# drprojects/superpoint_transformer

Hardware: AMD Instinct MI355X
Metric: Mpoints/s SPT fwd+bwd on S3DIS-scale NAG (higher is better)
Workload: dtype f32 (the reference's shipped matmul class - configs/train.yaml:60-61 `float32_matmul_precision: high` = TF32 / bf16x3 next to `precision: 32` - as bf16x3: matrix products on the bf16 pipe with split operands, attention and the backward of the fused layers and of the attention blocks' Linears hi*hi +

## Files before the change

include/spt_hip.h:

```cpp
#ifndef SPT_HIP_H
#define SPT_HIP_H

#include <stddef.h>
#include <stdint.h>

#ifdef __cplusplus
extern "C" {
#endif

typedef void* spt_stream_t;

enum spt_reduce_op {
  SPT_SUM = 0,
  SPT_MEAN = 1,
  SPT_MIN = 2,
  SPT_MAX = 3
};

typedef struct spt_gn_fwd_tables {
  const float* weight;
  const float* mean_scale;
  float eps;
  float* mean;
  float* rstd;
// ... 436 lines not shown
                                 float* gmean_scale, spt_stream_t stream);

int spt_fused_linear_supported(int K, int N);
int spt_fused_linear_use_split_bf16(int mode);
size_t spt_fused_linear_workspace_bytes(int K, int N);
int spt_fused_linear_fwd_f32(const float* x, int64_t r0, int64_t r1, int K, const float* W,
                             int N, const float* pre_am, const float* pre_scale,
                             const float* pre_bias, float pre_slope, float* h, double* total,
                             void* ws, size_t ws_bytes, spt_stream_t stream);
int spt_fused_linear_bwd_f32(const float* gy, const float* h, int64_t r0, int64_t r1, int N,
                             const float* am, const float* scale, const float* bias,
                             float slope, const float* c1, const float* c2, const float* c3,
                             const float* xprev, int K, const float* pre_am,
                             const float* pre_scale, const float* pre_bias, float pre_slope,
                             const float* W, float* gx, float* gW, int accumulate,
                             double* prev_total, void* ws, size_t ws_bytes, spt_stream_t stream);
int spt_fused_linear_pooled_supported(int K, int N);
int spt_fused_linear_pooled_supported_ex(int K, int N, int mode);
#define SPT_FMLP_BWD_REGISTER_STAGED 4
#define SPT_FMLP_H_BF16 8
#define SPT_FMLP_X_BF16 16
int spt_fused_linear_storage_supported(int K, int N);
int spt_fused_linear_bwd_use_dma(int on);
int spt_fused_linear_fwd_use_x3(int on);
int spt_fused_linear_fwd_ex_f32(const float* x, int64_t r0, int64_t r1, int K, const float* W,
                                int N, const float* pre_am, const float* pre_scale,
                                const float* pre_bias, float pre_slope, float* h, double* total,
                                int mode, void* ws, size_t ws_bytes, spt_stream_t stream);
int spt_fused_linear_bwd_ex_f32(const float* gy, const float* h, int64_t r0, int64_t r1, int N,
                                const float* am, const float* scale, const float* bias,
                                float slope, const float* c1, const float* c2, const float* c3,
                                const float* xprev, int K, const float* pre_am,
                                const float* pre_scale, const float* pre_bias, float pre_slope,
                                const float* W, float* gx, float* gW, int accumulate,
                                double* prev_total, int mode, void* ws, size_t ws_bytes,
                                spt_stream_t stream);
int spt_fused_linear_bwd_pooled_ex_f32(
    const float* gout, const int32_t* arg, const int32_t* perm, const int32_t* pos_seg,
    const float* h, int64_t p0, int64_t p1, int N, const float* am, const float* scale,
    const float* bias, float slope, const float* c1, const float* c2, const float* c3,
    const float* xprev, int K, const float* pre_am, const float* pre_scale, const float* pre_bias,
    float pre_slope, const float* W, float* gx, float* gW, int accumulate, double* prev_total,
    int mode, void* ws, size_t ws_bytes, spt_stream_t stream);
int spt_fused_linear_bwd_pooled_f32(
    const float* gout, const int32_t* arg, const int32_t* perm, const int32_t* pos_seg,
    const float* h, int64_t p0, int64_t p1, int N, const float* am, const float* scale,
// ... 116 lines not shown
```

superpoint_transformer_amd/_lib.py:

```python
import ctypes
import os

import torch

_HERE = os.path.dirname(os.path.abspath(__file__))
LIB_PATH = os.path.join(_HERE, "lib", "libspt_hip.so")

_c = ctypes
_i64 = _c.c_int64
_int = _c.c_int
_p = _c.c_void_p
_sz = _c.c_size_t
_f32 = _c.c_float
_f64 = _c.c_double

SIGNATURES = {
    "spt_version": (_int, []),
    "spt_last_error": (_c.c_char_p, []),
    "spt_csr_build_workspace_bytes": (_sz, [_i64, _i64]),
    "spt_csr_build": (_int, [_p, _i64, _i64, _p, _p, _p, _sz, _p]),
    "spt_csr_pos_seg": (_int, [_p, _i64, _i64, _p, _p]),
    "spt_csr_gather_i64_i32": (_int, [_p, _p, _i64, _p, _p]),
    "spt_segcsr_reduce_f32": (_int, [_int, _p, _p, _p, _i64, _i64, _int, _p, _p, _p]),
    "spt_segcsr_max_affine_f32": (_int, [_p, _p, _p, _i64, _i64, _int, _p, _p, _p, _f32, _p, _p, _p, _p]),
# ... 72 lines not shown
    "spt_spatial_order_workspace_bytes": (_sz, [_i64, _i64]),
    "spt_spatial_order": (_int, [_p, _i64, _f32, _p, _p, _p, _p, _sz, _p]),
    "spt_point_geof_csr_f32": (_int, [_p, _i64, _p, _p, _int, _int, _int, _p, _p]),
    "spt_vertical_edge_features_f32": (_int, [_p, _i64] + [_p] * 13 + [_p]),
    "spt_edge_affinity_features_f32": (_int, [_p, _i64, _int, _p, _p, _i64, _p, _p]),
    "spt_edge_affinity_features_bwd_f32": (_int, [_p, _p, _i64, _int, _p, _p, _i64, _p, _p]),
    "spt_scatter_pca_f32": (_int, [_p, _p, _p, _i64, _p, _p, _p]),
    "spt_neighbors_dense_to_csr_workspace_bytes": (_sz, [_i64]),
    "spt_neighbors_dense_to_csr": (_int, [_p, _i64, _int, _p, _p, _p, _p, _sz, _p]),
    "spt_horizontal_edge_features_f32": (_int, [_p, _i64, _i64, _p, _p, _p, _p, _p, _p, _p, _int,
                                                _p, _p, _p]),
    "spt_graphnorm_tables_f32": (_int, [_p, _int, _int, _p, _p, _f32, _p, _p, _p, _p, _p]),
    "spt_graphnorm_apply_f32": (_int, [_p, _p, _i64, _int, _int, _p, _p, _p, _f32, _p, _p]),
    "spt_graphnorm_bwd_stats_f32": (_int, [_p, _p, _p, _i64, _int, _int, _p, _p, _p, _f32, _p,
                                           _p, _sz, _p]),
    "spt_graphnorm_bwd_stats_sparse_workspace_bytes": (_sz, [_i64, _int, _int]),
    "spt_graphnorm_bwd_stats_sparse_f32": (_int, [_p, _p, _p, _p, _p, _i64, _i64, _int, _int, _p, _p,
                                                   _p, _f32, _p, _p, _sz, _p]),
    "spt_graphnorm_bwd_tables_f32": (_int, [_p, _int, _int, _p, _p, _p, _p, _p, _p, _p, _p, _p,
                                            _p, _p]),
    "spt_fused_linear_supported": (_int, [_int, _int]),
    "spt_fused_linear_use_split_bf16": (_int, [_int]),
    "spt_fused_linear_bwd_use_dma": (_int, [_int]),
    "spt_fused_linear_fwd_use_x3": (_int, [_int]),
    "spt_fused_linear_pooled_supported": (_int, [_int, _int]),
    "spt_fused_linear_bwd_pooled_f32": (_int, [_p, _p, _p, _p, _p, _i64, _i64, _int, _p, _p, _p, _f32,
                                               _p, _p, _p, _p, _int, _p, _p, _p, _f32, _p, _p, _p,
                                               _int, _p, _p, _sz, _p]),
    "spt_fused_linear_pooled_supported_ex": (_int, [_int, _int, _int]),
    "spt_fused_linear_fwd_ex_f32": (_int, [_p, _i64, _i64, _int, _p, _int, _p, _p, _p, _f32, _p, _p,
                                           _int, _p, _sz, _p]),
    "spt_fused_linear_bwd_ex_f32": (_int, [_p, _p, _i64, _i64, _int, _p, _p, _p, _f32, _p, _p, _p,
                                           _p, _int, _p, _p, _p, _f32, _p, _p, _p, _int, _p, _int, _p,
                                           _sz, _p]),
    "spt_fused_linear_bwd_pooled_ex_f32": (_int, [_p, _p, _p, _p, _p, _i64, _i64, _int, _p, _p, _p, _f32,
                                                  _p, _p, _p, _p, _int, _p, _p, _p, _f32, _p, _p, _p,
                                                  _int, _p, _int, _p, _sz, _p]),
    "spt_fused_linear_workspace_bytes": (_sz, [_int, _int]),
    "spt_fused_linear_fwd_runs_f32": (_int, [_p, _int, _p, _p, _p, _int, _int, _p, _int, _p, _p, _p,
                                             _f32, _p, _p, _int, _p, _sz, _p]),
    "spt_fused_linear_bwd_runs_f32": (_int, [_p, _p, _int, _p, _p, _p, _int, _int, _p, _p, _p, _f32,
                                             _p, _p, _p, _p, _int, _p, _p, _p, _f32, _p, _p, _p, _p,
                                             _int, _p, _sz, _p]),
    "spt_fused_linear_bwd_pooled_runs_f32": (_int, [_p, _p, _p, _p, _p, _int, _p, _p, _p, _int, _int,
                                                    _p, _p, _p, _f32, _p, _p, _p, _p, _int, _p, _p,
                                                    _p, _f32, _p, _p, _p, _p, _int, _p, _sz, _p]),
# ... 148 lines not shown
```

superpoint_transformer_amd/csrc/fused_mlp.hip:

```cpp
#include <math.h>
#include <stdlib.h>

#include "common.hpp"

namespace spt {
namespace fmlp {

typedef float f32x4 __attribute__((ext_vector_type(4)));
constexpr int WAVES = 4;
constexpr int TR = 16;
constexpr int MAX_BLOCKS = 1024;
constexpr int MAX_BWD_WAVES = 4096;

__device__ __forceinline__ double xg_sum_d(double v) {
  v += __shfl_xor(v, 16, 64);
  v += __shfl_xor(v, 32, 64);
  return v;
}
__device__ __forceinline__ void wave_sync_lds() {
  __builtin_amdgcn_fence(__ATOMIC_RELEASE, "wavefront");
  __builtin_amdgcn_wave_barrier();
  __builtin_amdgcn_fence(__ATOMIC_ACQUIRE, "wavefront");
}

// ... 1606 lines not shown
}

static int grid_for(int64_t rows, int per_cu) {
  const int64_t tiles = (rows + TR - 1) / TR;
  int64_t blocks = (tiles + WAVES - 1) / WAVES;
  const int64_t cap = 256 * per_cu;
  if (blocks > cap) blocks = cap;
  if (blocks < 1) blocks = 1;
  return (int)blocks;
}

}

bool fmlp_dma_supported(int K, int N);
int fmlp_dma_bwd_launch(bool pooled, bool lo, const float* gy, const float* h, FmlpRuns rt,
                        int64_t max_rows, int N, const float* am, const float* sc, const float* bs,
                        float slope, const float* c1, const float* c2, const float* c3,
                        const float* xprev, int K, const float* pam, const float* psc,
                        const float* pbs, float pslope, const float* W, float* gx,
                        float* gw_partial, double* pstat_partial, const int32_t* perm,
                        const int32_t* pos_seg, const float* gout, const int32_t* arg,
                        hipStream_t stream, bool s16 = false, int* gw_tabs = nullptr,
                        const float* x0 = nullptr, const float* fshift = nullptr,
                        float* fold_partial = nullptr, int K0 = 0);
bool fmlp_dma_fold_supported(int K0, int K, int N);
int fmlp_fold_len(int K, int K0);
}

using namespace spt;
using namespace spt::fmlp;

#define SPT_FMLP_SHAPES(X) X(3, 2) X(5, 2) X(8, 2) X(8, 4) X(16, 4) X(16, 8) X(17, 4) X(33, 4)

static std::atomic<int> g_fmlp_mode{1};
static inline int fmlp_mode_of(int mode) { return mode < 0 ? (int)g_fmlp_mode : (mode & 3); }
static std::atomic<int> g_fmlp_x3{[] { const char* e = getenv("SPT_FMLP_X3"); return e ? (atoi(e) != 0) : 1; }()};
extern "C" int spt_fused_linear_fwd_use_x3(int on) {
  const int prev = g_fmlp_x3;
  if (on >= 0) g_fmlp_x3 = on != 0;
  return prev;
}
static std::atomic<int> g_fmlp_dma{1};
static inline bool fmlp_dma_of(int mode) { return g_fmlp_dma != 0 && !(mode >= 0 && (mode & 4)); }
extern "C" int spt_fused_linear_bwd_use_dma(int on) {
  const int prev = g_fmlp_dma;
  if (on >= 0) g_fmlp_dma = on != 0;
  return prev;
}
// ... 304 lines not shown
    else if (g_fmlp_mode == 3)                                                                   \
      bwd_kernel_bf<a, b, false, NWB, false><<<grid, NWB * 64, 0, stream>>>(                     \
          gy, h, 0, 0, am, scale, bias, slope, c1, c2, c3, xprev, K, pre_am, pre_scale,          \
          pre_bias, pre_slope, W, nullptr, gwp, nullptr, rt);                                    \
    else if (g_fmlp_split_bf16 && gx)                                                            \
      bwd_kernel_bf<a, b, true, NWB, true><<<grid, NWB * 64, 0, stream>>>(                       \
          gy, h, 0, 0, am, scale, bias, slope, c1, c2, c3, xprev, K, pre_am, pre_scale,          \
          pre_bias, pre_slope, W, gx, gwp, pstp, rt);                                            \
    else if (g_fmlp_split_bf16)                                                                  \
      bwd_kernel_bf<a, b, false, NWB, true><<<grid, NWB * 64, 0, stream>>>(                      \
          gy, h, 0, 0, am, scale, bias, slope, c1, c2, c3, xprev, K, pre_am, pre_scale,          \
          pre_bias, pre_slope, W, nullptr, gwp, nullptr, rt);                                    \
    else if (gx)                                                                                 \
      bwd_kernel<a, b, true, NWV, big><<<grid, NWV * 64, 0, stream>>>(                           \
          gy, h, 0, 0, am, scale, bias, slope, c1, c2, c3, xprev, K, pre_am, pre_scale,          \
          pre_bias, pre_slope, W, gx, gwp, pstp, rt);                                            \
    else                                                                                         \
      bwd_kernel<a, b, false, NWV, big><<<grid, NWV * 64, 0, stream>>>(                          \
          gy, h, 0, 0, am, scale, bias, slope, c1, c2, c3, xprev, K, pre_am, pre_scale,          \
          pre_bias, pre_slope, W, nullptr, gwp, nullptr, rt);                                    \
  }
  float* fold_tabs = nullptr;
  float* fold_shift = nullptr;
  int per_run = 0;
  int gw_tabs = 0;
  const bool h16 = mode >= 0 && (mode & SPT_FMLP_H_BF16), x16 = mode >= 0 && (mode & SPT_FMLP_X_BF16);
  if (h16 || x16) {
    SPT_CHECK_ARG(g_fmlp_mode == 3 && h16 && spt_fused_linear_storage_supported(K, N) &&
                  (!x16 || K % 16 == 0),
                  "bf16 activation storage: bf16 matrix mode, a built shape, h stored as bf16");
#define XSP(a, b)                                                                                \
  if (pooled && k4 == a && nbk == b) {                                                           \
    constexpr bool big = (a * b >= 32);                                                          \
    constexpr int NWB = (a * b > 128) ? 4 : (big ? 8 : 4);                                       \
    gx_ = cap_grid(grid_for_nw(max_rows, (a * b > 128) ? 1 : (big ? ((a * b <= 32) ? 2 : 1) : 4), NWB), NWB); \
    nwv = NWB;                                                                                   \
    gw_tabs = gx_ * (fmlp_bf_wg_reduce(a, b, NWB) ? 1 : NWB);                                    \
    const dim3 grid((unsigned)gx_, (unsigned)nr);                                                \
    if (x16)                                                                                     \
      bwd_kernel_bf<a, b, true, NWB, false, true, false, true, true><<<grid, NWB * 64, 0, stream>>>( \
          nullptr, h, 0, 0, am, scale, bias, slope, c1, c2, c3, xprev, K, pre_am, pre_scale,     \
          pre_bias, pre_slope, W, gx, gwp, pstp, rt, perm, pos_seg, gout, arg);                  \
    else                                                                                         \
      bwd_kernel_bf<a, b, true, NWB, false, true, false, true, false><<<grid, NWB * 64, 0, stream>>>( \
          nullptr, h, 0, 0, am, scale, bias, slope, c1, c2, c3, xprev, K, pre_am, pre_scale,     \
          pre_bias, pre_slope, W, gx, gwp, pstp, rt, perm, pos_seg, gout, arg);                  \
// ... 4 lines not shown
    constexpr int NWV = big ? 8 : 4;                                                             \
    constexpr int NWB = (a * b > 128) ? 4 : NWV;                                                 \
    gx_ = cap_grid(grid_for_nw(max_rows, (a * b > 128) ? 1 : (big ? ((a * b <= 32) ? 2 : 1) : 4), NWB), NWB); \
    nwv = NWB;                                                                                   \
    gw_tabs = gx_ * (fmlp_bf_wg_reduce(a, b, NWB) ? 1 : NWB);                                    \
    const dim3 grid((unsigned)gx_, (unsigned)nr);                                                \
    if (gx && x16)                                                                               \
      bwd_kernel_bf<a, b, true, NWB, false, false, false, true, true><<<grid, NWB * 64, 0, stream>>>( \
          gy, h, 0, 0, am, scale, bias, slope, c1, c2, c3, xprev, K, pre_am, pre_scale,          \
          pre_bias, pre_slope, W, gx, gwp, pstp, rt);                                            \
    else if (gx)                                                                                 \
      bwd_kernel_bf<a, b, true, NWB, false, false, false, true, false><<<grid, NWB * 64, 0, stream>>>( \
          gy, h, 0, 0, am, scale, bias, slope, c1, c2, c3, xprev, K, pre_am, pre_scale,          \
          pre_bias, pre_slope, W, gx, gwp, pstp, rt);                                            \
    else if (x16)                                                                                \
      bwd_kernel_bf<a, b, false, NWB, false, false, false, true, true><<<grid, NWB * 64, 0, stream>>>( \
          gy, h, 0, 0, am, scale, bias, slope, c1, c2, c3, xprev, K, pre_am, pre_scale,          \
          pre_bias, pre_slope, W, nullptr, gwp, nullptr, rt);                                    \
    else                                                                                         \
      bwd_kernel_bf<a, b, false, NWB, false, false, false, true, false><<<grid, NWB * 64, 0, stream>>>( \
          gy, h, 0, 0, am, scale, bias, slope, c1, c2, c3, xprev, K, pre_am, pre_scale,          \
          pre_bias, pre_slope, W, nullptr, gwp, nullptr, rt);                                    \
  }
    if (x16 && gx && fmlp_dma_of(mode) && fmlp_dma_supported(K, N)) {
      per_run = fmlp_dma_bwd_launch(pooled, false, gy, h, rt, max_rows, N, am, scale, bias, slope, c1,
                                    c2, c3, xprev, K, pre_am, pre_scale, pre_bias, pre_slope, W, gx,
                                    gwp, pstp, perm, pos_seg, gout, arg, stream, true, &gw_tabs);
    } else {
      SPT_FMLP_ST_POOLED_SHAPES(XSP)
      SPT_FMLP_ST_SHAPES(XSD)
      per_run = gx_ * nwv;
    }
#undef XSP
#undef XSD
  } else if (fold_x0) {
    constexpr size_t FOLD_MAX_TABS = 1024;
    const int flen = fmlp_fold_len(K, fold_K0);
    SPT_CHECK_ARG((FOLD_MAX_TABS * ((size_t)N * K + flen) + FMLP_MAX_RUNS * FOLD_SHIFT_LD) * 4 <=
                  (size_t)MAX_BWD_WAVES * N * K * 4, "fold: tables do not fit the workspace");
    fold_tabs = gwp + FOLD_MAX_TABS * N * K;
    fold_shift = fold_tabs + FOLD_MAX_TABS * flen;
    fold_shift_kernel<<<num_graphs, 1024, 0, stream>>>(fold_x0, fold_K0, rt, fold_shift);
    if (fmlp_dma_of(mode) && fmlp_dma_fold_supported(fold_K0, K, N)) {
      per_run = fmlp_dma_bwd_launch(false, true, gy, h, rt, max_rows, N, am, scale, bias, slope, c1, c2,
                                    c3, xprev, K, pre_am, pre_scale, pre_bias, pre_slope, W, nullptr,
                                    gwp, pstp, nullptr, nullptr, nullptr, nullptr, stream, false,
                                    &gw_tabs, fold_x0, fold_shift, fold_tabs, fold_K0);
    } else if (fold_K0 == 18 && k4 == 8 && nbk == 2) {
      constexpr int NWB = 4;
      gx_ = cap_grid(grid_for_nw(max_rows, 4, NWB), NWB);
      nwv = NWB;
      gw_tabs = gx_;
      const dim3 grid((unsigned)gx_, (unsigned)nr);
      bwd_kernel_bf<8, 2, true, NWB, true, false, false, false, false, 18><<<grid, NWB * 64, 0, stream>>>(
          gy, h, 0, 0, am, scale, bias, slope, c1, c2, c3, xprev, K, pre_am, pre_scale, pre_bias,
          pre_slope, W, nullptr, gwp, pstp, rt, nullptr, nullptr, nullptr, nullptr, fold_x0, fold_shift,
          fold_tabs);
      per_run = gx_ * nwv;
    }
    SPT_CHECK_ARG((size_t)gw_tabs * nr <= FOLD_MAX_TABS, "fold: more tables than the workspace layout holds");
  } else if (g_fmlp_split_bf16 && gx && fmlp_dma_of(mode) && fmlp_dma_supported(K, N)) {
    per_run = fmlp_dma_bwd_launch(pooled, g_fmlp_mode != 3, gy, h, rt, max_rows, N, am, scale, bias,
                                  slope, c1, c2, c3, xprev, K, pre_am, pre_scale, pre_bias, pre_slope,
                                  W, gx, gwp, pstp, perm, pos_seg, gout, arg, stream, false, &gw_tabs);
  } else if (pooled) {
    SPT_FMLP_POOLED_SHAPES(XP)
    per_run = gx_ * nwv;
  } else {
    SPT_FMLP_SHAPES(X)
    per_run = gx_ * nwv;
  }
#undef X
#undef XP
  SPT_CHECK_ARG(per_run > 0, "no kernel for this shape");
  FmlpFold fd = {};
  if (fold_x0) {
    fd.tabs = fold_tabs;
    fd.shift = fold_shift;
    fd.gW0 = fold_gW0;
    fd.W0 = fold_W0;
    fd.am0 = pre_am;
    fd.K0 = fold_K0;
    fd.ZP = fold_zp(fold_K0);
    fd.grp = fmlp_groups(rt, num_graphs, gw_tabs);
  }
  bwd_post_launch(gwp, gw_tabs * nr, N * K, gW, accumulate, pst, fmlp_groups(rt, num_graphs, per_run), K,
                  num_graphs, prev_total, prev_norm, stream, fold_x0 ? &fd : nullptr);
// ... 109 lines not shown
extern "C" int spt_fused_linear_bwd_runs_gn_f32(
    const float* gy, const float* h, int nruns, const int64_t* run_r0, const int64_t* run_r1,
    const int32_t* run_graph, int num_graphs, int N, const float* am, const float* scale,
    const float* bias, float slope, const float* c1, const float* c2, const float* c3,
    const float* xprev, int K, const float* pre_am, const float* pre_scale, const float* pre_bias,
    float pre_slope, const float* W, float* gx, float* gW, double* prev_total, int mode, void* ws,
    size_t ws_bytes, const spt_gn_bwd_tables* prev_norm, spt_stream_t stream_) {
  FmlpRuns rt;
  int64_t max_rows;
  const char* err = fmlp_make_runs(nruns, run_r0, run_r1, run_graph, num_graphs, &rt, &max_rows);
  SPT_CHECK_ARG(!err, err ? err : "");
  SPT_CHECK_ARG(prev_norm, "null norm descriptor");
  return fmlp_bwd_impl(false, gy, nullptr, nullptr, nullptr, nullptr, h, rt, max_rows, num_graphs, N,
                       am, scale, bias, slope, c1, c2, c3, xprev, K, pre_am, pre_scale, pre_bias,
                       pre_slope, W, gx, gW, 0, prev_total, mode, ws, ws_bytes, (hipStream_t)stream_,
                       prev_norm);
}

extern "C" int spt_fused_linear_bwd_fold_supported(int K0, int K, int N, int mode) {
  const int m = fmlp_mode_of(mode);
  if (mode >= 0 && (mode & (SPT_FMLP_H_BF16 | SPT_FMLP_X_BF16))) return 0;
  return m == 1 && g_fmlp_x3 &&
         ((fmlp_dma_of(mode) && fmlp_dma_fold_supported(K0, K, N)) || (K0 == 18 && K == 32 && N == 32));
}
extern "C" int spt_fused_linear_bwd_runs_gn_fold_f32(
    const float* gy, const float* h, int nruns, const int64_t* run_r0, const int64_t* run_r1,
    const int32_t* run_graph, int num_graphs, int N, const float* am, const float* scale,
    const float* bias, float slope, const float* c1, const float* c2, const float* c3,
    const float* xprev, int K, const float* pre_am, const float* pre_scale, const float* pre_bias,
    float pre_slope, const float* W, float* gW, int mode, void* ws, size_t ws_bytes,
    const spt_gn_bwd_tables* prev_norm, const float* x0, int K0, const float* W0, float* gW0,
    spt_stream_t stream_) {
  FmlpRuns rt;
  int64_t max_rows;
  const char* err = fmlp_make_runs(nruns, run_r0, run_r1, run_graph, num_graphs, &rt, &max_rows);
  SPT_CHECK_ARG(!err, err ? err : "");
  SPT_CHECK_ARG(prev_norm && x0 && W0 && gW0, "null pointer");
  return fmlp_bwd_impl(false, gy, nullptr, nullptr, nullptr, nullptr, h, rt, max_rows, num_graphs, N,
                       am, scale, bias, slope, c1, c2, c3, xprev, K, pre_am, pre_scale, pre_bias,
                       pre_slope, W, nullptr, gW, 0, nullptr, mode, ws, ws_bytes, (hipStream_t)stream_,
                       prev_norm, x0, K0, W0, gW0);
}

namespace spt {
bool fpool_supported(int K, int N);
int fpool_gram_len(int K);
// ... 151 lines not shown
```

superpoint_transformer_amd/csrc/fused_mlp_dma.hip:

```cpp
#include <math.h>

#include "common.hpp"

#ifndef SPT_FDMA_SKIP
#define SPT_FDMA_SKIP 0
#endif

namespace spt {
namespace fdma {

typedef float f32x4 __attribute__((ext_vector_type(4)));
typedef __bf16 bf16x8 __attribute__((ext_vector_type(8)));
typedef __bf16 bf16x4 __attribute__((ext_vector_type(4)));
typedef short s16x4 __attribute__((ext_vector_type(4)));
constexpr int TR = 16;

__device__ __forceinline__ double xg_sum_d(double v) {
  v += __shfl_xor(v, 16, 64);
  v += __shfl_xor(v, 32, 64);
  return v;
}
__device__ __forceinline__ void lds_order() {
  __builtin_amdgcn_fence(__ATOMIC_RELEASE, "wavefront");
  __builtin_amdgcn_wave_barrier();
  __builtin_amdgcn_fence(__ATOMIC_ACQUIRE, "wavefront");
}
__device__ __forceinline__ void lds_dma16(const void* g, float* lds) {
#if SPT_FDMA_SKIP & 32
  return;
#endif
  const unsigned a = __builtin_amdgcn_readfirstlane(
      (unsigned)(size_t)((__attribute__((address_space(3))) void*)lds));
  asm volatile("s_mov_b32 m0, %0\n\ts_nop 0\n\tglobal_load_lds_dwordx4 %1, off"
               :: "s"(a), "v"(g) : "memory");
}
__device__ __forceinline__ void wait_vm0() {
  asm volatile("s_waitcnt vmcnt(0)" ::: "memory");
  __builtin_amdgcn_fence(__ATOMIC_ACQUIRE, "wavefront");
}
__device__ __forceinline__ void wait_lds() {
  asm volatile("s_waitcnt lgkmcnt(0)" ::: "memory");
}
__device__ __forceinline__ int opaque(int v) {
  asm volatile("" : "+v"(v));
  return v;
}
template <int NV, typename V>
__device__ __forceinline__ void split_bf16(const float (&x)[NV], V& hi, V& lo) {
#pragma unroll
  for (int i = 0; i < NV; ++i) {
    const __bf16 h = (__bf16)x[i];
    hi[i] = h;
    lo[i] = (__bf16)(x[i] - (float)h);
  }
}
template <bool LO>
// ... 22 lines not shown
  int r = __builtin_amdgcn_readlane(v, base);
#pragma unroll
  for (int j = 1; j < R; ++j) r = (sel == j) ? __builtin_amdgcn_readlane(v, base + j) : r;
  return r;
}

constexpr int fold_len(int K, int K0) { return (K + (K0 + 16) / 16 * 16) * ((K0 + 16) / 16 * 16); }
template <int K, int N, int NW, int OCC, bool LO, bool POOLED, bool S16 = false, int FK0 = 0>
__global__ __launch_bounds__(NW * 64, OCC) void bwd_dma_kernel(
    const float* __restrict__ gy, const float* __restrict__ h, int64_t r0, int64_t r1,
    const float* __restrict__ am, const float* __restrict__ sc, const float* __restrict__ bs,
    float slope, const float* __restrict__ c1, const float* __restrict__ c2,
    const float* __restrict__ c3, const float* __restrict__ xprev,
    const float* __restrict__ pam, const float* __restrict__ psc, const float* __restrict__ pbs,
    float pslope, const float* __restrict__ W, float* __restrict__ gx,
    float* __restrict__ gw_partial, double* __restrict__ pstat_partial,
    const int32_t* __restrict__ perm, const int32_t* __restrict__ pos_seg,
    const float* __restrict__ gout, const int32_t* __restrict__ arg, FmlpRuns rt,
    const float* __restrict__ x0 = nullptr, const float* __restrict__ fshift = nullptr,
    float* __restrict__ fold_partial = nullptr) {
  constexpr bool FOLD = FK0 > 0;
  constexpr int FOLD_K0 = FK0;
  static_assert(!FOLD || (!POOLED && !S16), "the fold reads dense f32 rows");
  static_assert(!FOLD || (FK0 % 4 == 0 && FK0 < 16 && TR * FK0 * 4 <= 1024), "x0 tile: one DMA block, one k block");
  constexpr int NC = N / 4, KC = K / 4, NBK = N / 16, KB = K / 16, NS = N / 32;
  if (rt.n > 0) {
    const int run_ = blockIdx.y, gph_ = rt.g[run_];
    r0 = rt.r0[run_];
    r1 = rt.r1[run_];
    am += (size_t)gph_ * N; sc += (size_t)gph_ * N;
    c1 += (size_t)gph_ * N; c2 += (size_t)gph_ * N; c3 += (size_t)gph_ * N;
    if (pam) { pam += (size_t)gph_ * K; psc += (size_t)gph_ * K; }
    gw_partial += (size_t)run_ * gridDim.x * N * K;
    if (pstat_partial) pstat_partial += (size_t)run_ * gridDim.x * NW * (2 * K + 1);
    if constexpr (FOLD) {
      fshift += (size_t)gph_ * 32;
      fold_partial += (size_t)run_ * gridDim.x * fold_len(K, FK0);
    }
  }
  constexpr int HI = TR * NC / 64, XI = TR * KC / 64;
  constexpr int RH = 64 / NC;
  constexpr int NSEG = RH;
  constexpr int LDT = N + 8;
  constexpr int W_H = TR * N, W_X = TR * K, W_G = POOLED ? NSEG * N : 0;
  static_assert(K % 16 == 0 && N % 32 == 0 && (TR * NC) % 64 == 0 && (TR * KC) % 64 == 0, "shape");
  __shared__ __attribute__((aligned(16))) float lw[NW][W_H + W_X + 2 * W_G];
  __shared__ __attribute__((aligned(16))) __bf16 wt_hi[K * LDT];
  __shared__ __attribute__((aligned(16))) __bf16 wt_lo[LO ? K * LDT : 8];
  __shared__ __attribute__((aligned(16))) float pt[3 * K];
  __shared__ __attribute__((aligned(16))) float x0b[FOLD ? NW : 1][FOLD ? 256 : 4];
  __shared__ float fsh[16];
  const int lane = threadIdx.x & 63;
  const int wid = __builtin_amdgcn_readfirstlane(threadIdx.x >> 6);
  const int g = lane >> 4, c = lane & 15;
  float* HB = lw[wid];
  float* XB = HB + W_H;
  float* GO = XB + W_X;
  int* AR = reinterpret_cast<int*>(GO + W_G);
  const bool pre = pam != nullptr;
  for (int i = threadIdx.x; i < K * N; i += NW * 64) {
    const int k = i / N, n = i - k * N;
    const float w = W[(size_t)n * K + k];
    const __bf16 hh = (__bf16)w;
    wt_hi[k * LDT + n] = hh;
    if constexpr (LO) wt_lo[k * LDT + n] = (__bf16)(w - (float)hh);
  }
  if constexpr (FOLD) {
    if (threadIdx.x < 16) fsh[threadIdx.x] = threadIdx.x < FOLD_K0 ? fshift[threadIdx.x] : 0.f;
  }
  for (int i = threadIdx.x; i < K; i += NW * 64) {
    pt[i] = pre ? pam[i] : 0.f;
    pt[K + i] = pre ? psc[i] : 1.f;
    pt[2 * K + i] = pre ? pbs[i] : 0.f;
  }
  __syncthreads();

  f32x4 C3[NBK][KB];
#pragma unroll
  for (int nb = 0; nb < NBK; ++nb)
#pragma unroll
    for (int kb = 0; kb < KB; ++kb) C3[nb][kb] = (f32x4){0.f, 0.f, 0.f, 0.f};
  double p1[KB], p2[KB];
#pragma unroll
  for (int kb = 0; kb < KB; ++kb) p1[kb] = p2[kb] = 0.0;
  f32x4 FA[FOLD ? KB : 1], FG = (f32x4){0.f, 0.f, 0.f, 0.f};
#pragma unroll
  for (int kb = 0; kb < (FOLD ? KB : 1); ++kb) FA[kb] = (f32x4){0.f, 0.f, 0.f, 0.f};
  float* X0B = x0b[FOLD ? wid : 0];

  const int64_t ntiles = (r1 - r0 + TR - 1) / TR;
  const int64_t wave = (int64_t)blockIdx.x * NW + wid;
  const int64_t nwaves = (int64_t)gridDim.x * NW;

  const float4 t_am = *reinterpret_cast<const float4*>(am + 4 * (lane % NC));
  const float4 t_sc = *reinterpret_cast<const float4*>(sc + 4 * (lane % NC));
  const float4 t_bs = *reinterpret_cast<const float4*>(bs + 4 * (lane % NC));
  const float4 t_c1 = *reinterpret_cast<const float4*>(c1 + 4 * (lane % NC));
  const float4 t_c2 = *reinterpret_cast<const float4*>(c2 + 4 * (lane % NC));
  const float4 t_c3 = *reinterpret_cast<const float4*>(c3 + 4 * (lane % NC));
  int ln = opaque(lane);
  auto gh1 = [&](float hh, float gg, float aa, float ss, float bb, float q1, float q2, float q3) {
    const float o = hh - aa;
    if (slope != 1.f) {
      const float y = fmaf(o, ss, bb);
      gg = (y > 0.f) ? gg : gg * slope;
    }
    return fmaf(q1, gg, -fmaf(q2, o, q3));
  };
  auto gh_of = [&](const float4& hv, const float4& gv) {
    return make_float4(gh1(hv.x, gv.x, t_am.x, t_sc.x, t_bs.x, t_c1.x, t_c2.x, t_c3.x),
// ... 46 lines not shown
                  HB + W_H / 2 + 256 * i);
    } else {
      const float* hb = POOLED ? h : h + row0 * N;
#pragma unroll
      for (int i = 0; i < HI; ++i) {
        const int rr7 = (hi + RH * i) & 7;
        lds_dma16(hb + (int64_t)pick(rid_l, RH * i) * N + 4 * (n4 ^ rr7), HB + 256 * i);
      }
    }
    if constexpr (POOLED) {
      const int cnt = (int)((r1 - row0) < TR ? (r1 - row0) : TR);
      const int s0 = __builtin_amdgcn_readlane(seg_l, 0);
      const int s1 = __builtin_amdgcn_readfirstlane(__shfl(seg_l, cnt - 1, 64));
      const int64_t sgm = (s0 + hi < s1) ? s0 + hi : s1;
      lds_dma16(gout + sgm * N + 4 * n4, GO);
      lds_dma16(arg + sgm * N + 4 * n4, reinterpret_cast<float*>(AR));
    }
  };
  auto issue_x = [&](int64_t t, int rid_l) {
    if (t >= ntiles) return;
    const int64_t row0 = r0 + t * TR;
    if constexpr (FOLD) {
      const int cnt = (int)((r1 - row0) < TR ? (r1 - row0) : TR);
      const int last = cnt * FOLD_K0 - 4;
      lds_dma16(x0 + row0 * FOLD_K0 + (4 * ln < last ? 4 * ln : last), X0B);
    }
    if constexpr (S16) {
      const uint16_t* xb = reinterpret_cast<const uint16_t*>(xprev) + (POOLED ? 0 : row0 * K);
      const int x16 = ln / KC16, q16 = ln % KC16;
#pragma unroll
      for (int i = 0; i < XI16; ++i)
        lds_dma16(xb + (int64_t)pick_lane<RX16>(rid_l, RX16 * i, x16) * K + 8 * q16,
                  XB + W_X / 2 + 256 * i);
    } else {
      const float* xb = POOLED ? xprev : xprev + row0 * K;
      const int hx = ln / KC, px = ln % KC;
#pragma unroll
      for (int i = 0; i < XI; ++i) {
        const int rr = hx + RX * i;
        lds_dma16(xb + (int64_t)pickx(rid_l, RX * i) * K + 4 * (px ^ (4 * ((rr >> 2) & 1))), XB + 256 * i);
      }
    }
  };

  load_ids(wave);
  int rid_l = rid_n, seg_l = seg_n;
  issue_h(wave, rid_l, seg_l);
  issue_x(wave, rid_l);
// ... 104 lines not shown
    f32x4 CX[KB];
#pragma unroll
    for (int kb = 0; kb < KB; ++kb) CX[kb] = (f32x4){0.f, 0.f, 0.f, 0.f};
    if constexpr (!(SPT_FDMA_SKIP & 4)) {
#pragma unroll
      for (int sg = 0; sg < NS; ++sg) {
        const float4 a0 = *reinterpret_cast<const float4*>(HB + c * N + 4 * ((8 * sg + 2 * g) ^ (c & 7)));
        const float4 a1 = *reinterpret_cast<const float4*>(HB + c * N + 4 * ((8 * sg + 2 * g + 1) ^ (c & 7)));
        const float av[8] = {a0.x, a0.y, a0.z, a0.w, a1.x, a1.y, a1.z, a1.w};
        bf16x8 ah, alo;
        split_bf16<8>(av, ah, alo);
#pragma unroll
        for (int kb = 0; kb < KB; ++kb) {
          const bf16x8 bh = *reinterpret_cast<const bf16x8*>(wt_hi + (16 * kb + c) * LDT + 32 * sg + 8 * g);
          bf16x8 bl = bh;
          if constexpr (LO) bl = *reinterpret_cast<const bf16x8*>(wt_lo + (16 * kb + c) * LDT + 32 * sg + 8 * g);
          CX[kb] = mfma3_32<LO>(ah, alo, bh, bl, CX[kb]);
        }
      }
    }
    const int rid_cur = rid_l;
    wait_lds();
    issue_h(t + nwaves, rid_n, seg_n);
    bf16x4 X0h, X0l;
    if constexpr (FOLD) {
      float x0v[4];
#pragma unroll
      for (int r = 0; r < 4; ++r) {
        const int rr = 4 * g + r;
        const float xr = X0B[rr * FOLD_K0 + (c < FOLD_K0 ? c : 0)];
        const float one = (c == FOLD_K0) ? 1.f : 0.f;
        x0v[r] = (rr < cnt) ? ((c < FOLD_K0) ? xr - fsh[c] : one) : 0.f;
      }
      split_bf16<4>(x0v, X0h, X0l);
      FG = mfma3_16<LO>(X0h, X0l, X0h, X0l, FG);
    }
#pragma unroll
    for (int kb = 0; kb < KB; ++kb) {
      const int k = 16 * kb + c;
      float ggv[4] = {0.f, 0.f, 0.f, 0.f};
#pragma unroll
      for (int r = 0; r < 4; ++r) {
        float* xs = XB + (4 * g + r) * K + 4 * ((4 * kb + (c >> 2)) ^ (4 * (g & 1))) + (c & 3);
        const float v = CX[kb][r];
        if (!(SPT_FDMA_SKIP & 8) && pre) {
          const float o = *xs - pt[k];
          float gg = v;
          if (pslope != 1.f) {
            const float y = fmaf(o, pt[K + k], pt[2 * K + k]);
            gg = (y > 0.f) ? gg : gg * pslope;
          }
          p1[kb] += (double)gg;
          p2[kb] += (double)gg * (double)o;
          if constexpr (FOLD) ggv[r] = gg;
        }
        if constexpr (!FOLD) *xs = v;
      }
      if constexpr (FOLD) {
        bf16x4 ah, al;
        split_bf16<4>(ggv, ah, al);
        FA[kb] = mfma3_16<LO>(ah, al, X0h, X0l, FA[kb]);
      }
    }
    if constexpr (!FOLD) {
      lds_order();
#pragma unroll
      for (int i = 0; i < XI; ++i) {
        const int rr = hx + RX * i;
        const float4 v = *reinterpret_cast<const float4*>(XB + rr * K + 4 * px);
        const int64_t orow = POOLED ? (int64_t)pickx(rid_cur, RX * i) : row0 + rr;
        if (!(SPT_FDMA_SKIP & 16) && rr < cnt)
          *reinterpret_cast<float4*>(gx + orow * K + 4 * (px ^ (4 * ((rr >> 2) & 1)))) = v;
      }
    }
    wait_lds();
    issue_x(t + nwaves, rid_n);
    rid_l = rid_n;
    seg_l = seg_n;
    load_ids(t + 2 * nwaves);
  }
  wait_vm0();
  {
    constexpr int LDR = K + 4;
    static_assert(N * LDR <= NW * (W_H + W_X + 2 * W_G), "the table fits the tile buffers");
// ... 17 lines not shown
#pragma unroll
            for (int r = 0; r < 4; ++r) C3[nb][kb][r] += red[(16 * nb + 4 * g + r) * LDR + 16 * kb + c];
      }
      __syncthreads();
    }
  }
  if (wid == 0) {
    float* gwp = gw_partial + (size_t)blockIdx.x * N * K;
#pragma unroll
    for (int nb = 0; nb < NBK; ++nb)
#pragma unroll
      for (int kb = 0; kb < KB; ++kb)
#pragma unroll
        for (int r = 0; r < 4; ++r)
          gwp[(size_t)(16 * nb + 4 * g + r) * K + 16 * kb + c] = C3[nb][kb][r];
  }
  if constexpr (FOLD) {
    constexpr int FLN = fold_len(K, FK0);
    static_assert(FLN <= NW * (W_H + W_X + 2 * W_G), "the fold table fits the tile buffers");
    float* red = &lw[0][0];
    for (int w = 1; w < NW; ++w) {
      if (wid == w) {
#pragma unroll
        for (int r = 0; r < 4; ++r) {
#pragma unroll
          for (int kb = 0; kb < KB; ++kb) red[(16 * kb + 4 * g + r) * 16 + c] = FA[kb][r];
          red[(K + 4 * g + r) * 16 + c] = FG[r];
        }
      }
      __syncthreads();
      if (wid == 0) {
#pragma unroll
        for (int r = 0; r < 4; ++r) {
#pragma unroll
          for (int kb = 0; kb < KB; ++kb) FA[kb][r] += red[(16 * kb + 4 * g + r) * 16 + c];
          FG[r] += red[(K + 4 * g + r) * 16 + c];
        }
      }
      __syncthreads();
    }
    if (wid == 0) {
      float* fp = fold_partial + (size_t)blockIdx.x * FLN;
#pragma unroll
      for (int r = 0; r < 4; ++r) {
#pragma unroll
        for (int kb = 0; kb < KB; ++kb) fp[(16 * kb + 4 * g + r) * 16 + c] = FA[kb][r];
        fp[(K + 4 * g + r) * 16 + c] = FG[r];
      }
    }
  }
  if (pstat_partial) {
    double* pp = pstat_partial + (size_t)wave * (2 * K + 1);
#pragma unroll
    for (int kb = 0; kb < KB; ++kb) {
      const double a = xg_sum_d(p1[kb]), b = xg_sum_d(p2[kb]);
      if (g == 0) {
        pp[16 * kb + c] = a;
        pp[K + 16 * kb + c] = b;
      }
    }
    if (lane == 0) pp[2 * K] = (wave == 0) ? (double)(r1 - r0) : 0.0;
  }
}

}

bool fmlp_dma_fold_supported(int K0, int K, int N) {
  return K0 == 12 && K == 32 && N == 64;
}
int fmlp_fold_len(int K, int K0) { return fdma::fold_len(K, K0); }
bool fmlp_dma_supported(int K, int N) {
  return (K == 64 && N == 128) || (K == 32 && N == 64) || (K == 64 && N == 64);
}

bool fmlp_dma_fold_supported(int K0, int K, int N);
int fmlp_dma_bwd_launch(bool pooled, bool lo, const float* gy, const float* h, FmlpRuns rt,
                        int64_t max_rows, int N, const float* am, const float* sc, const float* bs,
                        float slope, const float* c1, const float* c2, const float* c3,
                        const float* xprev, int K, const float* pam, const float* psc,
                        const float* pbs, float pslope, const float* W, float* gx,
                        float* gw_partial, double* pstat_partial, const int32_t* perm,
                        const int32_t* pos_seg, const float* gout, const int32_t* arg,
                        hipStream_t stream, bool s16, int* gw_tabs, const float* x0,
                        const float* fshift, float* fold_partial, int K0) {
  using namespace fdma;
  const int64_t tiles = (max_rows + TR - 1) / TR;
  const int nr = rt.n < 1 ? 1 : rt.n;
  if (x0) {
    if (!fmlp_dma_fold_supported(K0, K, N) || pooled || s16 || !lo || !fshift || !fold_partial || !pam) return 0;
    int64_t blocks = (tiles + 8 - 1) / 8;
    const int64_t cap = (256 * 2) / nr > 1 ? (256 * 2) / nr : 1;
    if (blocks > cap) blocks = cap;
    if (blocks < 1) blocks = 1;
    const dim3 grid((unsigned)blocks, (unsigned)nr);
    bwd_dma_kernel<32, 64, 8, 4, true, false, false, 12><<<grid, 8 * 64, 0, stream>>>(
        gy, h, 0, 0, am, sc, bs, slope, c1, c2, c3, xprev, pam, psc, pbs, pslope, W, nullptr,
        gw_partial, pstat_partial, perm, pos_seg, gout, arg, rt, x0, fshift, fold_partial);
    if (gw_tabs) *gw_tabs = (int)blocks;
    return (int)blocks * 8;
  }
#define SPT_DMA_CASE(KK, NN, NWV, PER_CU, OCC)                                                        \
  if (K == KK && N == NN) {                                                                        \
    int64_t blocks = (tiles + NWV - 1) / NWV;                                                      \
                                      \
    const int64_t cap = (256 * PER_CU) / nr > 1 ? (256 * PER_CU) / nr : 1;                         \
    if (blocks > cap) blocks = cap;                                                                \
    if (blocks < 1) blocks = 1;                                                                    \
    const dim3 grid((unsigned)blocks, (unsigned)nr);                                               \
    if (s16 && pooled)                                                                             \
      bwd_dma_kernel<KK, NN, NWV, OCC, false, true, true><<<grid, NWV * 64, 0, stream>>>(          \
// ... 34 lines not shown
```

Before: 362.6.

## Route K=32,N=32 fused-linear backward and its K0=18 fold through the DMA kernel

Extends the LDS-DMA backward kernel to the 32x32 layer shape, including the GraphNorm fold with an 18-column input. Rows that do not fit one 16-byte DMA block are staged with per-dword global_load_lds, and the fold accumulators are tiled over multiple 16-column blocks. The grid is sized to match the existing non-DMA path. A route query entry point is exported so the host can tell which path a layer will take. The aim is to replace the register-staged backward for these small layers with the asynchronous DMA staging path, at the cost of more accumulator registers and extra single-dword DMA instructions.

```diff
diff --git a/include/spt_hip.h b/include/spt_hip.h
--- a/include/spt_hip.h
+++ b/include/spt_hip.h
@@ -482,6 +482,7 @@
 #define SPT_FMLP_X_BF16 16
 int spt_fused_linear_storage_supported(int K, int N);
 int spt_fused_linear_bwd_use_dma(int on);
+int spt_fused_linear_bwd_route(int K0, int K, int N, int mode);
 int spt_fused_linear_fwd_use_x3(int on);
 int spt_fused_linear_fwd_ex_f32(const float* x, int64_t r0, int64_t r1, int K, const float* W,
                                 int N, const float* pre_am, const float* pre_scale,
diff --git a/superpoint_transformer_amd/_lib.py b/superpoint_transformer_amd/_lib.py
--- a/superpoint_transformer_amd/_lib.py
+++ b/superpoint_transformer_amd/_lib.py
@@ -118,6 +118,7 @@
     "spt_fused_linear_supported": (_int, [_int, _int]),
     "spt_fused_linear_use_split_bf16": (_int, [_int]),
     "spt_fused_linear_bwd_use_dma": (_int, [_int]),
+    "spt_fused_linear_bwd_route": (_int, [_int, _int, _int, _int]),
     "spt_fused_linear_fwd_use_x3": (_int, [_int]),
     "spt_fused_linear_pooled_supported": (_int, [_int, _int]),
     "spt_fused_linear_bwd_pooled_f32": (_int, [_p, _p, _p, _p, _p, _i64, _i64, _int, _p, _p, _p, _f32,
diff --git a/superpoint_transformer_amd/csrc/fused_mlp.hip b/superpoint_transformer_amd/csrc/fused_mlp.hip
--- a/superpoint_transformer_amd/csrc/fused_mlp.hip
+++ b/superpoint_transformer_amd/csrc/fused_mlp.hip
@@ -1652,8 +1652,9 @@
                         const int32_t* pos_seg, const float* gout, const int32_t* arg,
                         hipStream_t stream, bool s16 = false, int* gw_tabs = nullptr,
                         const float* x0 = nullptr, const float* fshift = nullptr,
-                        float* fold_partial = nullptr, int K0 = 0);
+                        float* fold_partial = nullptr, int K0 = 0, int blocks32 = 0);
 bool fmlp_dma_fold_supported(int K0, int K, int N);
+bool fmlp_dma_dense_only(int K, int N);
 int fmlp_fold_len(int K, int K0);
 }
 
@@ -2004,6 +2005,8 @@
   }
   float* fold_tabs = nullptr;
   float* fold_shift = nullptr;
+  const int blocks32 = (K == 32 && N == 32) ? cap_grid(grid_for_nw(max_rows, 4, 4), 4) : 0;
+  const bool dma_dense_only = fmlp_dma_dense_only(K, N);
   int per_run = 0;
   int gw_tabs = 0;
   const bool h16 = mode >= 0 && (mode & SPT_FMLP_H_BF16), x16 = mode >= 0 && (mode & SPT_FMLP_X_BF16);
@@ -2054,7 +2057,7 @@
           gy, h, 0, 0, am, scale, bias, slope, c1, c2, c3, xprev, K, pre_am, pre_scale,          \
           pre_bias, pre_slope, W, nullptr, gwp, nullptr, rt);                                    \
   }
-    if (x16 && gx && fmlp_dma_of(mode) && fmlp_dma_supported(K, N)) {
+    if (x16 && gx && fmlp_dma_of(mode) && fmlp_dma_supported(K, N) && !dma_dense_only) {
       per_run = fmlp_dma_bwd_launch(pooled, false, gy, h, rt, max_rows, N, am, scale, bias, slope, c1,
                                     c2, c3, xprev, K, pre_am, pre_scale, pre_bias, pre_slope, W, gx,
                                     gwp, pstp, perm, pos_seg, gout, arg, stream, true, &gw_tabs);
@@ -2077,7 +2080,7 @@
       per_run = fmlp_dma_bwd_launch(false, true, gy, h, rt, max_rows, N, am, scale, bias, slope, c1, c2,
                                     c3, xprev, K, pre_am, pre_scale, pre_bias, pre_slope, W, nullptr,
                                     gwp, pstp, nullptr, nullptr, nullptr, nullptr, stream, false,
-                                    &gw_tabs, fold_x0, fold_shift, fold_tabs, fold_K0);
+                                    &gw_tabs, fold_x0, fold_shift, fold_tabs, fold_K0, blocks32);
     } else if (fold_K0 == 18 && k4 == 8 && nbk == 2) {
       constexpr int NWB = 4;
       gx_ = cap_grid(grid_for_nw(max_rows, 4, NWB), NWB);
@@ -2091,10 +2094,12 @@
       per_run = gx_ * nwv;
     }
     SPT_CHECK_ARG((size_t)gw_tabs * nr <= FOLD_MAX_TABS, "fold: more tables than the workspace layout holds");
-  } else if (g_fmlp_split_bf16 && gx && fmlp_dma_of(mode) && fmlp_dma_supported(K, N)) {
+  } else if (g_fmlp_split_bf16 && gx && fmlp_dma_of(mode) && fmlp_dma_supported(K, N) &&
+             !(pooled && dma_dense_only)) {
     per_run = fmlp_dma_bwd_launch(pooled, g_fmlp_mode != 3, gy, h, rt, max_rows, N, am, scale, bias,
                                   slope, c1, c2, c3, xprev, K, pre_am, pre_scale, pre_bias, pre_slope,
-                                  W, gx, gwp, pstp, perm, pos_seg, gout, arg, stream, false, &gw_tabs);
+                                  W, gx, gwp, pstp, perm, pos_seg, gout, arg, stream, false, &gw_tabs,
+                                  nullptr, nullptr, nullptr, 0, blocks32);
   } else if (pooled) {
     SPT_FMLP_POOLED_SHAPES(XP)
     per_run = gx_ * nwv;
@@ -2250,6 +2255,16 @@
   if (mode >= 0 && (mode & (SPT_FMLP_H_BF16 | SPT_FMLP_X_BF16))) return 0;
   return m == 1 && g_fmlp_x3 &&
          ((fmlp_dma_of(mode) && fmlp_dma_fold_supported(K0, K, N)) || (K0 == 18 && K == 32 && N == 32));
+}
+extern "C" int spt_fused_linear_bwd_route(int K0, int K, int N, int mode) {
+  const int m = fmlp_mode_of(mode);
+  if (K0 > 0) {
+    if (!spt_fused_linear_bwd_fold_supported(K0, K, N, mode)) return -1;
+    return fmlp_dma_of(mode) && fmlp_dma_fold_supported(K0, K, N);
+  }
+  if (mode >= 0 && (mode & (SPT_FMLP_H_BF16 | SPT_FMLP_X_BF16)))
+    return (mode & SPT_FMLP_X_BF16) && fmlp_dma_of(mode) && fmlp_dma_supported(K, N) && !fmlp_dma_dense_only(K, N);
+  return m >= 1 && fmlp_dma_of(mode) && fmlp_dma_supported(K, N);
 }
 extern "C" int spt_fused_linear_bwd_runs_gn_fold_f32(
     const float* gy, const float* h, int nruns, const int64_t* run_r0, const int64_t* run_r1,
diff --git a/superpoint_transformer_amd/csrc/fused_mlp_dma.hip b/superpoint_transformer_amd/csrc/fused_mlp_dma.hip
--- a/superpoint_transformer_amd/csrc/fused_mlp_dma.hip
+++ b/superpoint_transformer_amd/csrc/fused_mlp_dma.hip
@@ -32,6 +32,15 @@
   const unsigned a = __builtin_amdgcn_readfirstlane(
       (unsigned)(size_t)((__attribute__((address_space(3))) void*)lds));
   asm volatile("s_mov_b32 m0, %0\n\ts_nop 0\n\tglobal_load_lds_dwordx4 %1, off"
+               :: "s"(a), "v"(g) : "memory");
+}
+__device__ __forceinline__ void lds_dma4(const void* g, float* lds) {
+#if SPT_FDMA_SKIP & 32
+  return;
+#endif
+  const unsigned a = __builtin_amdgcn_readfirstlane(
+      (unsigned)(size_t)((__attribute__((address_space(3))) void*)lds));
+  asm volatile("s_mov_b32 m0, %0\n\ts_nop 0\n\tglobal_load_lds_dword %1, off"
                :: "s"(a), "v"(g) : "memory");
 }
 __device__ __forceinline__ void wait_vm0() {
@@ -100,7 +109,11 @@
   constexpr bool FOLD = FK0 > 0;
   constexpr int FOLD_K0 = FK0;
   static_assert(!FOLD || (!POOLED && !S16), "the fold reads dense f32 rows");
-  static_assert(!FOLD || (FK0 % 4 == 0 && FK0 < 16 && TR * FK0 * 4 <= 1024), "x0 tile: one DMA block, one k block");
+  constexpr int ZP = (FK0 + 16) / 16 * 16, ZB = ZP / 16;
+  constexpr bool X0_DMA16 = FK0 % 4 == 0 && TR * FK0 * 4 <= 1024;
+  constexpr int X0N = X0_DMA16 ? 1 : (TR * FK0 + 63) / 64;
+  constexpr int X0LEN = X0_DMA16 ? 256 : 64 * X0N;
+  static_assert(!FOLD || ZP <= 32, "the shift table holds 32 columns");
   constexpr int NC = N / 4, KC = K / 4, NBK = N / 16, KB = K / 16, NS = N / 32;
   if (rt.n > 0) {
     const int run_ = blockIdx.y, gph_ = rt.g[run_];
@@ -126,8 +139,8 @@
   __shared__ __attribute__((aligned(16))) __bf16 wt_hi[K * LDT];
   __shared__ __attribute__((aligned(16))) __bf16 wt_lo[LO ? K * LDT : 8];
   __shared__ __attribute__((aligned(16))) float pt[3 * K];
-  __shared__ __attribute__((aligned(16))) float x0b[FOLD ? NW : 1][FOLD ? 256 : 4];
-  __shared__ float fsh[16];
+  __shared__ __attribute__((aligned(16))) float x0b[FOLD ? NW : 1][FOLD ? X0LEN : 4];
+  __shared__ float fsh[32];
   const int lane = threadIdx.x & 63;
   const int wid = __builtin_amdgcn_readfirstlane(threadIdx.x >> 6);
   const int g = lane >> 4, c = lane & 15;
@@ -144,7 +157,7 @@
     if constexpr (LO) wt_lo[k * LDT + n] = (__bf16)(w - (float)hh);
   }
   if constexpr (FOLD) {
-    if (threadIdx.x < 16) fsh[threadIdx.x] = threadIdx.x < FOLD_K0 ? fshift[threadIdx.x] : 0.f;
+    if (threadIdx.x < 32) fsh[threadIdx.x] = threadIdx.x < FOLD_K0 ? fshift[threadIdx.x] : 0.f;
   }
   for (int i = threadIdx.x; i < K; i += NW * 64) {
     pt[i] = pre ? pam[i] : 0.f;
@@ -161,9 +174,14 @@
   double p1[KB], p2[KB];
 #pragma unroll
   for (int kb = 0; kb < KB; ++kb) p1[kb] = p2[kb] = 0.0;
-  f32x4 FA[FOLD ? KB : 1], FG = (f32x4){0.f, 0.f, 0.f, 0.f};
-#pragma unroll
-  for (int kb = 0; kb < (FOLD ? KB : 1); ++kb) FA[kb] = (f32x4){0.f, 0.f, 0.f, 0.f};
+  f32x4 FA[FOLD ? KB : 1][ZB], FG[ZB][ZB];
+#pragma unroll
+  for (int zb = 0; zb < ZB; ++zb) {
+#pragma unroll
+    for (int kb = 0; kb < (FOLD ? KB : 1); ++kb) FA[kb][zb] = (f32x4){0.f, 0.f, 0.f, 0.f};
+#pragma unroll
+    for (int za = 0; za < ZB; ++za) FG[za][zb] = (f32x4){0.f, 0.f, 0.f, 0.f};
+  }
   float* X0B = x0b[FOLD ? wid : 0];
 
   const int64_t ntiles = (r1 - r0 + TR - 1) / TR;
@@ -256,8 +274,17 @@
     const int64_t row0 = r0 + t * TR;
     if constexpr (FOLD) {
       const int cnt = (int)((r1 - row0) < TR ? (r1 - row0) : TR);
-      const int last = cnt * FOLD_K0 - 4;
-      lds_dma16(x0 + row0 * FOLD_K0 + (4 * ln < last ? 4 * ln : last), X0B);
+      if constexpr (X0_DMA16) {
+        const int last = cnt * FOLD_K0 - 4;
+        lds_dma16(x0 + row0 * FOLD_K0 + (4 * ln < last ? 4 * ln : last), X0B);
+      } else {
+        const int last = cnt * FOLD_K0 - 1;
+#pragma unroll
+        for (int i = 0; i < X0N; ++i) {
+          const int f = 64 * i + ln;
+          lds_dma4(x0 + row0 * FOLD_K0 + (f < last ? f : last), X0B + 64 * i);
+        }
+      }
     }
     if constexpr (S16) {
       const uint16_t* xb = reinterpret_cast<const uint16_t*>(xprev) + (POOLED ? 0 : row0 * K);
@@ -408,18 +435,26 @@
     const int rid_cur = rid_l;
     wait_lds();
     issue_h(t + nwaves, rid_n, seg_n);
-    bf16x4 X0h, X0l;
+    bf16x4 X0h[ZB], X0l[ZB];
     if constexpr (FOLD) {
-      float x0v[4];
-#pragma unroll
-      for (int r = 0; r < 4; ++r) {
-        const int rr = 4 * g + r;
-        const float xr = X0B[rr * FOLD_K0 + (c < FOLD_K0 ? c : 0)];
-        const float one = (c == FOLD_K0) ? 1.f : 0.f;
-        x0v[r] = (rr < cnt) ? ((c < FOLD_K0) ? xr - fsh[c] : one) : 0.f;
-      }
-      split_bf16<4>(x0v, X0h, X0l);
-      FG = mfma3_16<LO>(X0h, X0l, X0h, X0l, FG);
+#pragma unroll
+      for (int zb = 0; zb < ZB; ++zb) {
+        const int col = 16 * zb + c;
+        float x0v[4];
+#pragma unroll
+        for (int r = 0; r < 4; ++r) {
+          const int rr = 4 * g + r;
+          const float xr = X0B[rr * FOLD_K0 + (col < FOLD_K0 ? col : 0)];
+          const float one = (col == FOLD_K0) ? 1.f : 0.f;
+          x0v[r] = (rr < cnt) ? ((col < FOLD_K0) ? xr - fsh[col] : one) : 0.f;
+        }
+        split_bf16<4>(x0v, X0h[zb], X0l[zb]);
+      }
+#pragma unroll
+      for (int za = 0; za < ZB; ++za)
+#pragma unroll
+        for (int zb = 0; zb < ZB; ++zb)
+          FG[za][zb] = mfma3_16<LO>(X0h[za], X0l[za], X0h[zb], X0l[zb], FG[za][zb]);
     }
 #pragma unroll
     for (int kb = 0; kb < KB; ++kb) {
@@ -445,7 +480,8 @@
       if constexpr (FOLD) {
         bf16x4 ah, al;
         split_bf16<4>(ggv, ah, al);
-        FA[kb] = mfma3_16<LO>(ah, al, X0h, X0l, FA[kb]);
+#pragma unroll
+        for (int zb = 0; zb < ZB; ++zb) FA[kb][zb] = mfma3_16<LO>(ah, al, X0h[zb], X0l[zb], FA[kb][zb]);
       }
     }
     if constexpr (!FOLD) {
@@ -509,31 +545,40 @@
     for (int w = 1; w < NW; ++w) {
       if (wid == w) {
 #pragma unroll
-        for (int r = 0; r < 4; ++r) {
-#pragma unroll
-          for (int kb = 0; kb < KB; ++kb) red[(16 * kb + 4 * g + r) * 16 + c] = FA[kb][r];
-          red[(K + 4 * g + r) * 16 + c] = FG[r];
-        }
+        for (int zb = 0; zb < ZB; ++zb)
+#pragma unroll
+          for (int r = 0; r < 4; ++r) {
+#pragma unroll
+            for (int kb = 0; kb < KB; ++kb) red[(16 * kb + 4 * g + r) * ZP + 16 * zb + c] = FA[kb][zb][r];
+#pragma unroll
+            for (int za = 0; za < ZB; ++za) red[(K + 16 * za + 4 * g + r) * ZP + 16 * zb + c] = FG[za][zb][r];
+          }
       }
       __syncthreads();
       if (wid == 0) {
 #pragma unroll
-        for (int r = 0; r < 4; ++r) {
-#pragma unroll
-          for (int kb = 0; kb < KB; ++kb) FA[kb][r] += red[(16 * kb + 4 * g + r) * 16 + c];
-          FG[r] += red[(K + 4 * g + r) * 16 + c];
-        }
+        for (int zb = 0; zb < ZB; ++zb)
+#pragma unroll
+          for (int r = 0; r < 4; ++r) {
+#pragma unroll
+            for (int kb = 0; kb < KB; ++kb) FA[kb][zb][r] += red[(16 * kb + 4 * g + r) * ZP + 16 * zb + c];
+#pragma unroll
+            for (int za = 0; za < ZB; ++za) FG[za][zb][r] += red[(K + 16 * za + 4 * g + r) * ZP + 16 * zb + c];
+          }
       }
       __syncthreads();
     }
     if (wid == 0) {
       float* fp = fold_partial + (size_t)blockIdx.x * FLN;
 #pragma unroll
-      for (int r = 0; r < 4; ++r) {
-#pragma unroll
-        for (int kb = 0; kb < KB; ++kb) fp[(16 * kb + 4 * g + r) * 16 + c] = FA[kb][r];
-        fp[(K + 4 * g + r) * 16 + c] = FG[r];
-      }
+      for (int zb = 0; zb < ZB; ++zb)
+#pragma unroll
+        for (int r = 0; r < 4; ++r) {
+#pragma unroll
+          for (int kb = 0; kb < KB; ++kb) fp[(16 * kb + 4 * g + r) * ZP + 16 * zb + c] = FA[kb][zb][r];
+#pragma unroll
+          for (int za = 0; za < ZB; ++za) fp[(K + 16 * za + 4 * g + r) * ZP + 16 * zb + c] = FG[za][zb][r];
+        }
     }
   }
   if (pstat_partial) {
@@ -553,12 +598,13 @@
 }
 
 bool fmlp_dma_fold_supported(int K0, int K, int N) {
-  return K0 == 12 && K == 32 && N == 64;
+  return (K0 == 12 && K == 32 && N == 64) || (K0 == 18 && K == 32 && N == 32);
 }
 int fmlp_fold_len(int K, int K0) { return fdma::fold_len(K, K0); }
 bool fmlp_dma_supported(int K, int N) {
-  return (K == 64 && N == 128) || (K == 32 && N == 64) || (K == 64 && N == 64);
-}
+  return (K == 64 && N == 128) || (K == 32 && N == 64) || (K == 64 && N == 64) || (K == 32 && N == 32);
+}
+bool fmlp_dma_dense_only(int K, int N) { return K == 32 && N == 32; }
 
 bool fmlp_dma_fold_supported(int K0, int K, int N);
 int fmlp_dma_bwd_launch(bool pooled, bool lo, const float* gy, const float* h, FmlpRuns rt,
@@ -569,10 +615,30 @@
                         float* gw_partial, double* pstat_partial, const int32_t* perm,
                         const int32_t* pos_seg, const float* gout, const int32_t* arg,
                         hipStream_t stream, bool s16, int* gw_tabs, const float* x0,
-                        const float* fshift, float* fold_partial, int K0) {
+                        const float* fshift, float* fold_partial, int K0, int blocks32) {
   using namespace fdma;
   const int64_t tiles = (max_rows + TR - 1) / TR;
   const int nr = rt.n < 1 ? 1 : rt.n;
+  if (K == 32 && N == 32) {
+    if (pooled || s16 || blocks32 < 1) return 0;
+    const dim3 grid((unsigned)blocks32, (unsigned)nr);
+    if (x0) {
+      if (!fmlp_dma_fold_supported(K0, K, N) || !lo || !fshift || !fold_partial || !pam) return 0;
+      bwd_dma_kernel<32, 32, 4, 4, true, false, false, 18><<<grid, 4 * 64, 0, stream>>>(
+          gy, h, 0, 0, am, sc, bs, slope, c1, c2, c3, xprev, pam, psc, pbs, pslope, W, nullptr,
+          gw_partial, pstat_partial, perm, pos_seg, gout, arg, rt, x0, fshift, fold_partial);
+    } else if (lo) {
+      bwd_dma_kernel<32, 32, 4, 4, true, false><<<grid, 4 * 64, 0, stream>>>(
+          gy, h, 0, 0, am, sc, bs, slope, c1, c2, c3, xprev, pam, psc, pbs, pslope, W, gx,
+          gw_partial, pstat_partial, perm, pos_seg, gout, arg, rt);
+    } else {
+      bwd_dma_kernel<32, 32, 4, 4, false, false><<<grid, 4 * 64, 0, stream>>>(
+          gy, h, 0, 0, am, sc, bs, slope, c1, c2, c3, xprev, pam, psc, pbs, pslope, W, gx,
+          gw_partial, pstat_partial, perm, pos_seg, gout, arg, rt);
+    }
+    if (gw_tabs) *gw_tabs = blocks32;
+    return blocks32 * 4;
+  }
   if (x0) {
     if (!fmlp_dma_fold_supported(K0, K, N) || pooled || s16 || !lo || !fshift || !fold_partial || !pam) return 0;
     int64_t blocks = (tiles + 8 - 1) / 8;
```

Result: faster. 367.9, median of 6 (+1.5%).
